# zrjer/Sparse-Matrix-Factorization-Library

Hardware: AMD Instinct MI355X
Metric: numeric-factorization GFLOP/s (supernodal Cholesky) (higher is better)
Workload: dtype f64; 1 GPU; 3D 7-point Laplacian 128^3 SPD Cholesky fp64, geometric ND, devSlotSize 8694792192; n=2097152, nnz_input=8339456, nsuper=35419, factor_doubles=3787034536, parallelism=single GPU, grid_rule=BASELINE config

## Files before the change

### sparse-matrix-factorization-library_amd/csrc/sf_chol_plan.hip

```cpp
#include <sparseframe_hip.h>

#include <algorithm>
#include <time.h>
#include <cmath>
#include <cstdio>
#include <cstdlib>
#include <cstring>
#include <string>
#include <vector>

#include "sf_plan_internal.h"
#include "sf_symbolic.h"

static bool elapsed_ms(float* ms, hipEvent_t a, hipEvent_t b) {
    if (hipEventElapsedTime(ms, a, b) == hipSuccess) return true;
    (void)hipGetLastError();
    return false;
}

extern "C" {

int sf_device_count(void) {
    int n = 0;
    if (hipGetDeviceCount(&n) != hipSuccess) return 0;
// ... 206 lines not shown
                break;
            case 1: sf::launch_trsm(p->d_trsm + L.first, L.count, p->d_Lsx, pc.pivinv, st); break;
            case 7: {
                const int g = (int)L.first;
                const int upto = p->ooc_wait.empty() ? g - 2 : p->ooc_wait[(size_t)g];
                for (int w = std::max(0, g - 2); w <= upto && w < g; ++w) {
                    std::unique_lock<std::mutex> lk(p->dl_mu);
                    p->dl_cv.wait(lk, [&] { return p->dl_abort || p->dl_group_left[(size_t)w].load() <= 0; });
                    if (p->dl_abort) return SF_ERR_HIP;
                }
                if (g >= 2 && p->ooc_buf > 0) {
                    const size_t off = (size_t)(g & 1) * (size_t)p->ooc_buf, nb = (size_t)p->ooc_buf * sizeof(double);
                    HIP_TRY(hipMemsetAsync(p->d_Lsx + off, 0, nb, st));
                    if (p->lu) HIP_TRY(hipMemsetAsync(p->d_Lsx + p->xC + off, 0, nb, st));
                }
                if (p->ooc_top_mode >= 1)
                    for (const auto& z : p->ooc_zero[(size_t)g]) {
                        HIP_TRY(hipMemsetAsync(p->d_Lsx + z.first, 0, (size_t)z.second * sizeof(double), st));
                        if (p->lu) HIP_TRY(hipMemsetAsync(p->d_Lsx + p->xC + z.first, 0, (size_t)z.second * sizeof(double), st));
                    }
                assemble(p->d_loadmask + (size_t)g * (size_t)p->nsuper, st);
                break;
            }
            case 6: {
                int64_t lo, hi;
                launch_window(L, L.count, &lo, &hi);
                sf::launch_update_small(p->d_probs, p->d_stasks + L.first + lo, (int)(hi - lo), p->d_Lsx, p->d_relmap, st);
                break;
            }
            case 5:
                sf::launch_step(p->d_steps + L.first, L.count, p->lu ? 1 : 0, p->d_Lsx, p->d_flags, p->epoch, p->d_info, p->d_tinv,
                                p->d_info + 1 + L.ticket, pc, st);
                break;
            case 2:
            case 3:
            case 4: {
                int64_t w0, w1;
                launch_window(L, L.units, &w0, &w1);
                const uint32_t u0 = (uint32_t)w0, u1 = (uint32_t)w1;
                sf::launch_gemm(p->d_probs, p->d_gtasks + L.first, p->d_ktprefix + L.prefix_first, L.count, u0, u1,
                                L.kind == 3 ? 1 : 0, p->d_Lsx, p->d_relmap, p->gemm_dynamic ? p->d_info + 1 + L.ticket : nullptr, st,
                                (L.whole_tiles && !L.split) ? 1 : 0, 0);
                break;
            }
        }
        if (p->profiling) { kinds.push_back(L.kind); mark(); }
        if (p->dl_active) HIP_TRY(dl_publish(p, li + 1));
    }
    if (last && !p->capturing) HIP_TRY(hipEventRecord(p->ev1, st));
    HIP_TRY(hipGetLastError());
    if (p->profiling) {
        HIP_TRY(hipStreamSynchronize(st));
        if (first) {
            p->last_load_ms = p->last_panel_ms = p->last_update_ms = 0;
            for (double& v : p->last_kind_ms) v = 0;
        }
        float ms = 0;
        if (first && !evs.empty() && elapsed_ms(&ms, p->ev0, evs[0])) p->last_load_ms = ms;
        FILE* dump = nullptr;
        if (const char* path = getenv("SF_PROFILE_DUMP")) dump = fopen(path, first ? "w" : "a");
        if (dump && first) fprintf(dump, "launch,kind,tasks,units,flops,ms\n");
        for (size_t k = 0; k + 1 < evs.size(); ++k) {
            if (!elapsed_ms(&ms, evs[k], evs[k + 1])) continue;
            if (kinds[k] == 3) p->last_update_ms += ms; else if (kinds[k] != 6) p->last_panel_ms += ms;
            p->last_kind_ms[kinds[k]] += ms;
            if (dump) {
// ... 761 lines not shown
    if (!p || !name) return -1;
    const std::string k(name);
    if (k == "levels") return p->nlevels;
    if (k == "last_solve_ms") return p->last_solve_ms;
    if (k == "last_solve_many_ms") return p->last_solve_many_ms;
    if (k == "bytes_solve_many") return (double)p->bytes_solve_many;
    if (k == "solve_many_width") return (double)sf::SVM_W;
    if (k == "bytes_selinv") return (double)p->bytes_selinv;
    if (k == "last_selinv_ms") return p->last_selinv_ms;
    if (k == "flops_selinv") return p->flops_selinv;
    if (k == "selinv_valid") return (p->d_sel && p->sel_gen == p->factor_gen) ? 1.0 : 0.0;
    if (k == "perturbed_pivots") return (double)p->last_perturbed;
    if (k == "pivot_tol") return p->piv_tol;
    if (k == "last_to_host_ms") return p->last_to_host_ms;
    if (k == "download_pieces") return (double)p->dl_pieces.size();
    if (k == "top_doubles") return (double)p->top_size;
    if (k == "stored_doubles") return (double)p->xC;
    if (k == "launches") return (double)p->launches.size();
    if (k == "gemm_tasks") return (double)p->n_gemm_tasks;
    if (k == "update_pairs") return (double)p->n_pairs;
    if (k == "flops_exec") return p->flops_exec;
    if (k == "flops_update") return p->flops_update;
    if (k == "flops_panel_gemm") return p->flops_panel_gemm;
    if (k == "scatter_elems") return p->scatter_elems;
    if (k == "bytes_device") return (double)p->bytes_device;
    if (k == "last_ms") return p->last_ms;
    if (k == "last_load_ms") return p->last_load_ms;
    if (k == "last_panel_ms") return p->last_panel_ms;
    if (k == "last_update_ms") return p->last_update_ms;
    if (k == "last_potrf_ms") return p->last_kind_ms[0];
    if (k == "last_trsm_ms") return p->last_kind_ms[1];
    if (k == "last_inner_gemm_ms") return p->last_kind_ms[2];
    if (k == "last_outer_gemm_ms") return p->last_kind_ms[4];
    if (k == "last_step_ms") return p->last_kind_ms[5];
    if (k == "last_small_update_ms") return p->last_kind_ms[6];
    if (k == "flops_update_small") return p->flops_update_small;
    if (k == "flops_outer_gemm") return p->flops_outer_gemm;
    if (k == "flops_tiles") return p->flops_tiles;
    if (k == "flops_tiles_update") return p->flops_tiles_update;
    return -1;
}

}

void sf_solve_step_fwd(sf_chol_plan* p, size_t k, const double* base, int* sync, int* tickets, hipStream_t st) {
    const auto& s = p->solve_steps[k];
    const int32_t* piv = (p->lu && p->piv_tol > 0.0) ? p->d_piv : nullptr;
    const int unit = p->lu ? 1 : 0;
    int* tk = tickets + sf_chol_plan::SOLVE_TICKETS * k;
    if (s.small) {
        sf::launch_solve_small_fwd(p->d_solve + s.fwd_first, s.ndiag, base, p->d_Lsi, p->d_x, unit, piv, st);
    } else {
        sf::launch_solve_fwd(p->d_solve + s.fwd_first, s.fwd_count, s.big, base, p->d_Lsi, p->d_x, unit, piv, sync, tk, p->d_solve_sync, st);
    }
}

void sf_solve_step_bwd(sf_chol_plan* p, size_t k, const double* base, int* sync, int* tickets, hipStream_t st) {
    const auto& s = p->solve_steps[k];
    int* tk = tickets + sf_chol_plan::SOLVE_TICKETS * k;
    if (s.small) {
        sf::launch_solve_small_bwd(p->d_solve + s.bwd_first, s.ndiag, base, p->d_Lsi, p->d_x, st);
    } else if (p->solve_bwd_fused) {
        sf::launch_solve_bwd(p->d_solve + s.bwd_first, s.count, s.big, base, p->d_Lsi, p->d_x, sync, tk + 1, p->d_solve_sync, st, p->d_solveT);
    } else {
        sf::launch_solve_bwd(p->d_solve + s.bwd_first, s.nrows_tasks, 0, base, p->d_Lsi, p->d_x, sync, tk + 1, p->d_solve_sync, st);
        sf::launch_solve_bwd(p->d_solve + s.bwd_first + s.nrows_tasks, s.count - s.nrows_tasks, s.big, base, p->d_Lsi, p->d_x, sync, tk + 2,
                             p->d_solve_sync, st, p->d_solveT);
// ... 128 lines not shown
```

### sparse-matrix-factorization-library_amd/csrc/sf_kernels.h

```cpp
#pragma once
#include <hip/hip_runtime.h>
#include <cstdint>

#include <cstdlib>
static inline const char* sf_exp_env(const char* name) {
#ifdef SF_EXPERIMENTS
    return getenv(name);
#else
    (void)name;
    return nullptr;
#endif
}

namespace sf {

constexpr int NB = 64;
constexpr int OUTER_NB = 512;
constexpr int TRSM_ROWS = 256;
constexpr int ST_ROWS = 64;
constexpr int GEMM_BM = 128;
constexpr int GEMM_BN = 128;
constexpr int GEMM_BK = 16;
constexpr int GEMM_WAVES = 8;
constexpr int GEMM_THREADS = 64 * GEMM_WAVES;
// ... 54 lines not shown
};

struct StepTask {
    int64_t panel;
    int64_t xpanel;
    int32_t ld, J, diag, b;
    int32_t row0, nrows;
    int32_t flag;
    int32_t mode;
    int32_t slot;
    int32_t next_b;
    int32_t first_col;
    int32_t pad;
};

void launch_build_loadmap(const int64_t* Lp, const int32_t* Li, int32_t n, const int32_t* Super, const int32_t* SuperMap,
                          const int64_t* Lsip, const int32_t* Lsi, const int64_t* Lsxp, int64_t base, int skip_diag, int64_t* map, hipStream_t st);
void launch_loadmap_drop(const int64_t* drop, int64_t count, int64_t* map, hipStream_t st);
void launch_load_mapped(const double* Lx, const int64_t* map, int64_t nnz, double* Lsx, hipStream_t st);
void launch_load_panels(const int64_t* Lp, const int32_t* Li, const double* Lx, int32_t n,
                        const int32_t* Super, const int32_t* SuperMap, const int64_t* Lsip, const int32_t* Lsi,
                        const int64_t* Lsxp, double* Lsx, int skip_diag, const int8_t* load_mask, hipStream_t st);
void launch_potrf(const PotrfTask* tasks, int ntasks, double* Lsx, int* info, hipStream_t st);
void launch_getrf(const PotrfTask* tasks, int ntasks, double* Lsx, int64_t u_shift, int* info, PivotCtl pc, hipStream_t st);
struct FillTile { int64_t xp; int32_t nsrow, r0, c0, cb, ce; };
void launch_factor_hash(const int32_t* Super, const int64_t* Lsip, const int64_t* Xp, const int64_t* RefXp, int32_t nsuper,
                        const double* PL, const double* PU, int lu, int64_t total, unsigned long long* H, hipStream_t st);
void launch_lu_fill_u11(const FillTile* tiles, int64_t ntiles, double* PL, const double* PU, hipStream_t st);
void launch_pack_lu(const int32_t* Super, const int64_t* Lsip, const int64_t* Xp, const int64_t* RefXp, int32_t nsuper,
                    const double* PL, const double* PU, double* out, int64_t e_begin, int64_t e_end, hipStream_t st);
void launch_trsm(const TrsmTask* tasks, int ntasks, double* Lsx, const int32_t* pivinv, hipStream_t st);
void launch_step(const StepTask* tasks, int ntasks, int lu, double* Lsx, int* flags, int epoch, int* info, double* tinv, int* ticket,
                 PivotCtl pc, hipStream_t st);
void launch_build_relmaps(const GemmProb* probs, int nprobs, const int32_t* Lsi, int32_t* RelMap, hipStream_t st);

void launch_gemm(const GemmProb* probs, const GemmTask* tasks, const uint32_t* kt_prefix, int ntasks, uint32_t u_lo, uint32_t u_hi,
                 int mode, double* Lsx, const int32_t* RelMap, int* ticket, hipStream_t st, int whole_tiles = 0, int grid_cap = 0);

void launch_update_small(const GemmProb* probs, const GemmTask* tasks, int ntasks, double* Lsx, const int32_t* RelMap, hipStream_t st);

struct SolveTask {
    int64_t panel;
    int64_t rows;
    int32_t ld, diag, b;
    int32_t row0, nrows;
    int32_t first_col;
    int32_t flag;
    int32_t expect;
    int64_t tdiag;
};
void launch_solve_small_fwd(const SolveTask* t, int nt, const double* Lsx, const int32_t* Lsi, double* x, int unit, const int32_t* pivpos,
                            hipStream_t st);
void launch_solve_small_bwd(const SolveTask* t, int nt, const double* Lsx, const int32_t* Lsi, double* x, hipStream_t st);
void launch_solve_fwd(const SolveTask* t, int nt, int big, const double* Lsx, const int32_t* Lsi, double* x, int unit, const int32_t* pivpos,
                      int* sync, int* ticket, int* info, hipStream_t st);
void launch_solve_bwd(const SolveTask* t, int nt, int big, const double* Lsx, const int32_t* Lsi, double* x, int* sync, int* ticket, int* info,
                      hipStream_t st, const double* Tbase = nullptr);
void launch_solve_transpose_diag(const SolveTask* tasks, const int64_t* list, int64_t ntasks, const double* Lsx, double* T, hipStream_t st);

constexpr int SVM_W = 16;
void launch_solve_many_small_fwd(const SolveTask* t, int nt, const double* Lsx, const int32_t* Lsi, double* x, int unit,
                                 const int32_t* pivpos, hipStream_t st);
void launch_solve_many_small_bwd(const SolveTask* t, int nt, const double* Lsx, const int32_t* Lsi, double* x, hipStream_t st);
void launch_solve_many_fwd(const SolveTask* t, int nt, int big, const double* Lsx, const int32_t* Lsi, double* x, int unit,
                           const int32_t* pivpos, int* sync, int* ticket, int* info, hipStream_t st);
void launch_solve_many_bwd(const SolveTask* t, int nt, int big, const double* Lsx, const int32_t* Lsi, double* x, int* sync, int* ticket,
// ... 23 lines not shown
```

### sparse-matrix-factorization-library_amd/csrc/sf_kernels.hip

```cpp
#include "sf_kernels.h"
#include <cstdlib>
#include "sf_wave.h"

namespace sf {

typedef double double4_t __attribute__((ext_vector_type(4)));
typedef double double2_t __attribute__((ext_vector_type(2), aligned(8)));

__device__ __forceinline__ int lower_bound_i32(const int32_t* __restrict__ a, int n, int32_t key) {
    int lo = 0, hi = n;
    while (lo < hi) {
        const int mid = (lo + hi) >> 1;
        if (a[mid] < key) lo = mid + 1; else hi = mid;
    }
    return lo;
}

__global__ void __launch_bounds__(256)
k_load_panels(const int64_t* __restrict__ Lp, const int32_t* __restrict__ Li, const double* __restrict__ Lx, int32_t n,
              const int32_t* __restrict__ Super, const int32_t* __restrict__ SuperMap,
              const int64_t* __restrict__ Lsip, const int32_t* __restrict__ Lsi,
              const int64_t* __restrict__ Lsxp, double* __restrict__ Lsx, int skip_diag,
              const int8_t* __restrict__ load_mask) {
    const int32_t j = blockIdx.x * blockDim.x + threadIdx.x;
// ... 1597 lines not shown
        g_exp_stamps[(size_t)gridDim.x * 256 + blockIdx.x * 4 + 3] = wall_clock64();
    }
#endif
}

#ifndef SF_LU_STEP_WGS
#define SF_LU_STEP_WGS 3
#endif
#ifndef SF_GEMM_MIN_UNITS_DEFAULT
#define SF_GEMM_MIN_UNITS_DEFAULT 16
#endif
#ifndef SF_POTRF_PW
#define SF_POTRF_PW 16
#endif
constexpr int ST_ULD = ST_ROWS + 1;
constexpr int ST_KC = 32;
constexpr int ST_XLD = ST_ROWS + 16;
constexpr int ST_SPIN_LIMIT = 1 << 22;

#ifdef SF_EXP_STEP_STAMPS
__device__ unsigned long long* g_step_stamps = nullptr;
void exp_set_step_stamps(unsigned long long* p) { (void)hipMemcpyToSymbol(HIP_SYMBOL(g_step_stamps), &p, sizeof(p)); }
#define ST_STAMP(slot) do { if (is_diag && tid == 0 && g_step_stamps) g_step_stamps[slot] = wall_clock64(); } while (0)
#else
#define ST_STAMP(slot) do { } while (0)
#endif

__device__ __forceinline__ double ld_agent(const double* p) {
    return __hip_atomic_load(p, __ATOMIC_RELAXED, __HIP_MEMORY_SCOPE_AGENT);
}
__device__ __forceinline__ int ld_agent(const int* p) {
    return __hip_atomic_load(p, __ATOMIC_RELAXED, __HIP_MEMORY_SCOPE_AGENT);
}

template <bool LU>
__global__ void __launch_bounds__(256, LU ? SF_LU_STEP_WGS : 3)
k_step(const StepTask* __restrict__ tasks, double* __restrict__ Lsx, int* __restrict__ flags, int epoch, int* __restrict__ info,
       double* __restrict__ tinv, int* __restrict__ ticket, PivotCtl pc) {
    constexpr int SMEM = 2 * ST_KC * ST_XLD;
    __shared__ __attribute__((aligned(16))) double smem[SMEM];
    static_assert(NB == ST_ROWS && NB == 64, "one wavefront per 64 x 64 tile");
    static_assert(NB * ST_ULD <= SMEM && NB * NB + 4 * 256 <= SMEM, "phases must fit the LDS array");
    double* __restrict__ U = smem;
    double (*Dt)[NB] = reinterpret_cast<double (*)[NB]>(smem);

    __shared__ int s_ticket;
    const int tid = threadIdx.x, lane = tid & 63, wave = tid >> 6;
#ifdef SF_EXP_STEP_STAMPS
    const unsigned long long st_entry = wall_clock64();
#endif
    if (tid == 0) s_ticket = __hip_atomic_fetch_add(ticket, 1, __ATOMIC_RELAXED, __HIP_MEMORY_SCOPE_AGENT);
    __syncthreads();
    const StepTask t = tasks[__builtin_amdgcn_readfirstlane(s_ticket)];
    const bool is_pre = LU && (t.mode & 2);
    const bool is_diag = t.row0 == t.diag && !is_pre;
#ifdef SF_EXP_STEP_STAMPS
    if (is_diag && tid == 0 && g_step_stamps) g_step_stamps[0] = st_entry;
#endif
    ST_STAMP(1);
    const int fr = lane & 15, fk = lane >> 4;
    const int64_t ld = t.ld;
    const int b = t.b, nrows = t.nrows;
    const int nhp = ((is_pre ? t.diag - NB : t.diag) - t.J) / NB;
    double* __restrict__ Ag = Lsx + t.panel + t.row0 + (int64_t)t.diag * ld;
    const double* __restrict__ Dg = Lsx + t.xpanel + t.diag + (int64_t)t.diag * ld;

    double4_t acc[4];
#pragma unroll
    for (int a = 0; a < 4; ++a) acc[a] = (double4_t){0.0, 0.0, 0.0, 0.0};

    if (nhp > 0) {
        double (*Xs)[ST_KC][ST_XLD] = reinterpret_cast<double (*)[ST_KC][ST_XLD]>(smem);
        const int nch = 2 * nhp;
        const int prow = 2 * (tid & 31), pk0 = tid >> 5;
        const double* __restrict__ xp = Lsx + t.xpanel + t.diag + (int64_t)t.J * ld + ((prow < b) ? prow : 0);
        const double* __restrict__ yp = Lsx + t.panel + t.row0 + (int64_t)(t.J + fk) * ld + min(16 * wave + fr, nrows - 1);
        const int nhalf = 2 * nch;
        double2_t rx[2][4];
        double fy[4][4];
        auto load_x = [&](int sel, int h) __attribute__((always_inline)) {
            const int hc = min(h, nch - 1);
#pragma unroll
            for (int q = 0; q < 4; ++q) rx[sel][q] = *reinterpret_cast<const double2_t*>(xp + (int64_t)(hc * ST_KC + pk0 + 8 * q) * ld);
        };
        auto store_x = [&](int buf, int sel) __attribute__((always_inline)) {
#pragma unroll
            for (int q = 0; q < 4; ++q) *reinterpret_cast<double2_t*>(&Xs[buf][pk0 + 8 * q][prow]) = rx[sel][q];
        };
        auto load_y = [&](int slot, int hh) __attribute__((always_inline)) {
            const int hc = min(hh, nhalf - 1);
#pragma unroll
            for (int kk = 0; kk < 4; ++kk) fy[slot][kk] = yp[(int64_t)(hc * (ST_KC / 2) + 4 * kk) * ld];
        };
        auto compute = [&](int par, int h) __attribute__((always_inline)) {
            load_y((2 * par + 3) & 3, 2 * h + 3);
#pragma unroll
            for (int kk = 0; kk < 8; ++kk) {
                double a[4];
#pragma unroll
                for (int q = 0; q < 4; ++q) a[q] = Xs[par][4 * kk + fk][16 * q + fr];
                if (kk == 0) store_x(par ^ 1, par ^ 1);
                if (kk == 1) load_x(par ^ 1, h + 3);
                if (kk == 4) load_y(2 * par, 2 * h + 4);
#pragma unroll
                for (int q = 0; q < 4; ++q) acc[q] = __builtin_amdgcn_mfma_f64_16x16x4f64(a[q], fy[2 * par + (kk >> 2)][kk & 3], acc[q], 0, 0, 0);
            }
        };
        load_x(0, 0);
        load_x(1, 1);
        load_y(0, 0);
        load_y(1, 1);
        load_y(2, 2);
        store_x(0, 0);
        load_x(0, 2);
        __syncthreads();
        for (int hp = 0; hp < nhp; ++hp) {
            compute(0, 2 * hp);
            __syncthreads();
            compute(1, 2 * hp + 1);
            __syncthreads();
        }
    }

    if (is_pre) {
        double* __restrict__ Dw = Lsx + t.xpanel + t.diag + (int64_t)t.diag * ld;
// ... 34 lines not shown
#pragma unroll
            for (int i = 0; i < 16; ++i) {
                const int k = 16 * wave + i;
                if (lane > k) U[k * ST_ULD + lane] = (lane < b && k < b) ? blk[i] : 0.0;
            }
#pragma unroll
            for (int i = 0; i < 16; ++i) blk[i] = Dg[lc + (int64_t)min(16 * wave + i, b - 1) * ld];
#pragma unroll
            for (int i = 0; i < 16; ++i) {
                const int k = 16 * wave + i;
                if (lane >= k) U[lane * ST_ULD + k] = (lane < b && k < b) ? blk[i] : ((lane == k) ? 1.0 : 0.0);
            }
        }
        if (nhp > 0) {
            __syncthreads();
            const int ci = 16 * wave + fr;
#pragma unroll
            for (int q = 0; q < 4; ++q)
#pragma unroll
                for (int r = 0; r < 4; ++r) {
                    const int cj = 16 * q + fk + 4 * r;
                    if (ci < b && cj < b) U[cj * ST_ULD + ci] -= acc[q][r];
                }
        }
    } else if (is_diag) {
        const int ci = 16 * wave + fr;
#pragma unroll
        for (int q = 0; q < 4; ++q)
#pragma unroll
            for (int r = 0; r < 4; ++r) {
                const int cj = 16 * q + fk + 4 * r;
                const int cic = min(ci, nrows - 1), cjc = min(cj, b - 1);
                double v = (ci == cj) ? 1.0 : 0.0;
                const double av = Ag[cic + (int64_t)cjc * ld];
                if (ci < nrows && cj < b && cj <= ci) v = av - acc[q][r];
                U[cj * ST_ULD + ci] = v;
            }
    }

    if (LU && is_diag) {
        __shared__ int s_piv[NB], s_pos[NB];
        if (tid < NB) { s_pos[tid] = -1; s_piv[tid] = tid; }
        __syncthreads();
        ST_STAMP(2);
        bool bad = false, active = lane < b;
        int np = 0, pos = lane;
        bool nat_all = true;
#pragma unroll 1
        for (int q = 0; q < NB / 16; ++q) {
            const int c0 = 16 * q;
            if (wave == 0) {
                double a[16];
#pragma unroll
                for (int u = 0; u < 16; ++u) a[u] = U[(c0 + u) * ST_ULD + lane];
                bool done = false;
                if (nat_all) {
                    done = getrf_panel_natural<16>(a, lane, c0, b, pc.tol, pc.eps);
                    if (done) {
                        if (lane >= c0 && lane < c0 + 16) { active = false; s_piv[lane] = lane; }
                    } else {
#pragma unroll
                        for (int u = 0; u < 16; ++u) a[u] = U[(c0 + u) * ST_ULD + lane];
                    }
                }
                if (!done) {
                    nat_all = false;
                    getrf_panel_wave<true, 16>(a, lane, c0, b, pc.tol, pc.eps, bad, np, pos, active, s_piv);
// ... 242 lines not shown
            double dv[NB * NB / 256], tv[4];
#pragma unroll
            for (int i = 0; i < NB * NB / 256; ++i) {
                const int e = tid + 256 * i, k = e / NB, j = e % NB;
                dv[i] = ld_agent(Dg + min(j, b - 1) + (int64_t)min(k, b - 1) * ld);
            }
#pragma unroll
            for (int i = 0; i < 4; ++i) tv[i] = ld_agent(tsrc + tid + 256 * i);
#pragma unroll
            for (int i = 0; i < NB * NB / 256; ++i) {
                const int e = tid + 256 * i, k = e / NB, j = e % NB;
                Dt[k][j] = (j < b && k < j) ? dv[i] : 0.0;
            }
#pragma unroll
            for (int i = 0; i < 4; ++i) Tl[tid + 256 * i] = tv[i];
        }
        __syncthreads();
        const int ci = 16 * wave + fr;
#pragma unroll
        for (int q = 0; q < 4; ++q) {
            if (16 * q >= b) break;
            double4_t x = (double4_t){0.0, 0.0, 0.0, 0.0};
#pragma unroll
            for (int sg = 0; sg < 4; ++sg)
                x = __builtin_amdgcn_mfma_f64_16x16x4f64(Tl[q * 256 + (4 * sg + fk) * 16 + fr], rt[q][sg], x, 0, 0, 0);
#pragma unroll
            for (int qq = q + 1; qq < 4; ++qq)
#pragma unroll
                for (int sg = 0; sg < 4; ++sg)
                    rt[qq] = __builtin_amdgcn_mfma_f64_16x16x4f64(-Dt[16 * q + 4 * sg + fk][16 * qq + fr], x[sg], rt[qq], 0, 0, 0);
#pragma unroll
            for (int r = 0; r < 4; ++r) {
                const int cj = 16 * q + fk + 4 * r;
                if (ci < nrows && cj < b) Ag[ci + (int64_t)cj * ld] = x[r];
            }
            if (!LU && t.next_b > 0) {
                __syncthreads();
#pragma unroll
                for (int r = 0; r < 4; ++r) Dt[16 * q + fk + 4 * r][ci] = x[r];
            }
        }
        if (!LU && t.next_b > 0) {
            __syncthreads();
            double* __restrict__ Dn = Lsx + t.panel + t.row0 + (int64_t)t.row0 * ld;
            const int nb = t.next_b;
            for (int ct = 0; ct <= wave; ++ct) {
                double4_t d = (double4_t){0.0, 0.0, 0.0, 0.0};
#pragma unroll 4
                for (int sg = 0; sg < 16; ++sg)
                    d = __builtin_amdgcn_mfma_f64_16x16x4f64(Dt[4 * sg + fk][16 * ct + fr], Dt[4 * sg + fk][ci], d, 0, 0, 0);
                double old[4];
#pragma unroll
                for (int r = 0; r < 4; ++r) {
                    const int cj = 16 * ct + fk + 4 * r;
                    old[r] = Dn[min(ci, nb - 1) + (int64_t)min(cj, nb - 1) * ld];
                }
#pragma unroll
                for (int r = 0; r < 4; ++r) {
                    const int cj = 16 * ct + fk + 4 * r;
                    if (ci < nb && cj <= ci) Dn[ci + (int64_t)cj * ld] = old[r] - d[r];
                }
            }
        }
    }
}

void launch_step(const StepTask* tasks, int ntasks, int lu, double* Lsx, int* flags, int epoch, int* info, double* tinv, int* ticket,
                 PivotCtl pc, hipStream_t st) {
    if (ntasks <= 0) return;
    if (lu) hipLaunchKernelGGL(k_step<true>, dim3(ntasks), dim3(256), 0, st, tasks, Lsx, flags, epoch, info, tinv, ticket, pc);
    else hipLaunchKernelGGL(k_step<false>, dim3(ntasks), dim3(256), 0, st, tasks, Lsx, flags, epoch, info, tinv, ticket, pc);
}

__global__ void __launch_bounds__(256)
k_update_small(const GemmProb* __restrict__ probs, const GemmTask* __restrict__ tasks, int ntasks,
               double* __restrict__ Lsx, const int32_t* __restrict__ RelMap) {
    const int lane = threadIdx.x & 63;
    const int ti = __builtin_amdgcn_readfirstlane(blockIdx.x * 4 + (threadIdx.x >> 6));
    if (ti >= ntasks) return;
    const GemmTask tk = tasks[ti];
    const GemmProb pb = probs[tk.prob];
    const int fr = lane & 15, fk = lane >> 4;
    const int ci0 = tk.tm * SU_TM, cj0 = tk.tn * SU_TN;
    const int M = pb.M, N = pb.N, K = pb.K;
    const int64_t lda = pb.lda;
    const double* __restrict__ yq[4];
    const double* __restrict__ xq[2];
#pragma unroll
    for (int q = 0; q < 4; ++q) yq[q] = Lsx + pb.y_off + min(ci0 + 16 * q + fr, M - 1);
#pragma unroll
    for (int q = 0; q < 2; ++q) xq[q] = Lsx + pb.x_off + min(cj0 + 16 * q + fr, N - 1);

    double4_t acc[2][4];
#pragma unroll
    for (int a = 0; a < 2; ++a)
#pragma unroll
        for (int c = 0; c < 4; ++c) acc[a][c] = (double4_t){0.0, 0.0, 0.0, 0.0};

    const int nkk = (K + 3) >> 2;
    for (int kk0 = 0; kk0 < nkk; kk0 += 8) {
        double fa[8][2], fb[8][4];
#pragma unroll
        for (int kk = 0; kk < 8; ++kk) {
            const int k = 4 * (kk0 + kk) + fk;
// ... 161 lines not shown
```

### sparse-matrix-factorization-library_amd/csrc/sf_plan_build.hip

```cpp
#include <sparseframe_hip.h>

#include <algorithm>
#include <time.h>
#include <cmath>
#include <cstdio>
#include <cstdlib>
#include <cstring>
#include <vector>

#include "sf_plan_internal.h"
#include "sf_symbolic.h"

static thread_local double* t_offer_ptr = nullptr;
static thread_local size_t t_offer_bytes = 0;
extern "C" void sf_plan_offer_factor_buffer(double* ptr, size_t bytes) { t_offer_ptr = ptr; t_offer_bytes = bytes; }

struct PlanInput {
    sf_long n = 0, nsuper = 0;
    const sf_long *Super = nullptr, *SuperMap = nullptr, *Lsip = nullptr, *Lsi = nullptr, *Lsxp = nullptr;
    const sf_long *Lp = nullptr, *Li = nullptr, *Up = nullptr, *Ui = nullptr;
    bool lu = false;
    int device = 0;
    bool dry = false;
    const int32_t* phase_in = nullptr;
    int load_top = 1, rank = 0, nranks = 1;
    const uint32_t* top_mask = nullptr;
    const double* root_cum = nullptr;
    const int32_t* ooc_group = nullptr;
    int ooc_ngroups = 0, ooc_top_mode = 0;

    sf_long nscol(sf_long s) const { return Super[s + 1] - Super[s]; }
    sf_long nsrow(sf_long s) const { return Lsip[s + 1] - Lsip[s]; }
    bool ooc() const { return ooc_group != nullptr && ooc_ngroups > 1; }
    int sides() const { return lu ? 2 : 1; }
};

static bool exp_on(const char* name) {
    const char* env = sf_exp_env(name);
    return !(env && atoi(env) == 0);
}

struct PlanKnobs {
    bool trace = false;
    int su_maxk = sf::SU_MAXK;
    int64_t fuse_max = 32 * sf::GEMM_GRID;
    bool lookahead = true;
    bool use_graph = false;
    bool top_owner = false;
    bool solve_diagT = true, solve_bwd_ahead = true, solve_bwd_fused = true, solve_fwd_ahead = true, solve_fwd_far_first = true;
    int solve_far_wgs = 512, solve_far_groups = 8;
    int dl_workers = DL_WORKERS_DEFAULT, dl_workers_fresh = DL_WORKERS_FRESH;
    bool dl_host_wait = true;
    int64_t dl_slot = DL_SLOT_DEFAULT;
    bool dl_2d = true;
    bool dl_lu_pack = false;
    bool stream_priority = true;
    bool gemm_dynamic = true;
    double piv_tol = 0.0, piv_perturb = 0.0;
};

static PlanKnobs read_knobs() {
    PlanKnobs k;
    k.trace = getenv("SF_TRACE") != nullptr;
    if (const char* env = sf_exp_env("SF_SU_MAXK")) k.su_maxk = atoi(env);
    if (const char* env = getenv("SF_FUSE_MAX")) k.fuse_max = strtoll(env, nullptr, 10);
    if (const char* env = getenv("SF_LOOKAHEAD")) k.lookahead = atoi(env) != 0;
    if (const char* env = getenv("SF_GRAPH")) k.use_graph = atoi(env) != 0;
    if (const char* env = getenv("SF_TOP_OWNER")) k.top_owner = atoi(env) != 0;
    k.solve_diagT = exp_on("SF_SOLVE_DIAGT");
    k.solve_bwd_ahead = exp_on("SF_SOLVE_BWD_AHEAD");
    k.solve_bwd_fused = exp_on("SF_SOLVE_BWD_FUSED");
    k.solve_fwd_ahead = exp_on("SF_SOLVE_FWD_AHEAD");
    k.solve_fwd_far_first = exp_on("SF_SOLVE_FWD_FAR_FIRST");
    if (const char* env = sf_exp_env("SF_SOLVE_FAR_WGS")) k.solve_far_wgs = std::max(1, atoi(env));
    if (const char* env = sf_exp_env("SF_SOLVE_FAR_GROUPS")) k.solve_far_groups = std::max(1, std::min(64, atoi(env)));
    if (const char* env = getenv("SF_DL_WORKERS")) k.dl_workers = k.dl_workers_fresh = std::max(1, std::min(DL_WORKERS_MAX, atoi(env)));
    k.dl_host_wait = exp_on("SF_DL_HOST_WAIT");
    if (const char* env = getenv("SF_DL_SLOT_MB")) k.dl_slot = (int64_t)std::max(1, atoi(env)) << 17;
    k.dl_2d = exp_on("SF_DL_2D");
    if (const char* env = sf_exp_env("SF_DL_LU_PACK")) k.dl_lu_pack = atoi(env) != 0;
    k.stream_priority = exp_on("SF_STREAM_PRIORITY");
    k.gemm_dynamic = exp_on("SF_GEMM_DYNAMIC");
    if (const char* env = getenv("SF_LU_PIVOT_TOL")) {
        k.piv_tol = std::min(1.0, std::max(0.0, atof(env)));
        if (k.piv_tol > 0.0) k.piv_perturb = 1.4901161193847656e-08;
    }
    if (const char* env = getenv("SF_LU_PERTURB")) k.piv_perturb = std::max(0.0, atof(env));
    return k;
}

struct Layout {
    std::vector<int64_t> XP;
    std::vector<uint32_t> gmask;
    int64_t ushift = 0;
    uint32_t all_ranks = 1;
    int rank = 0;
    int group_idx(uint32_t m) const { return __builtin_popcount(m & ((1u << rank) - 1u)); }
};
// ... 456 lines not shown
        const int dnext = diag + sf::NB;
        for (sf_long s : LS.sn) {
            const int nscol = (int)in.nscol(s), nsrow = (int)in.nsrow(s);
            if (dnext >= nscol) continue;
            const int bn = std::min(sf::NB, nscol - dnext);
            steps.push_back(StepTask{XP[s], XP[s] + ushift, nsrow, J, dnext, bn, dnext, bn, -1, 2, 0, 0, (int32_t)in.Super[s], 0});
            sw.pre_updated[(size_t)s] = jo * 16 + ti + 1;
        }
    }
    size_t si = 0;
    for (sf_long s : LS.sn) {
        const int nscol = (int)in.nscol(s), nsrow = (int)in.nsrow(s);
        const int32_t fl = flag_of[si], sl = slot_of[si];
        ++si;
        if (fl < 0) continue;
        const int b = std::min(sf::NB, nscol - diag);
        for (int r = diag + b; r < nsrow; r += sf::ST_ROWS) {
            const int nr = std::min(sf::ST_ROWS, nsrow - r);
            if (!lu) {
                const int nb = (r < std::min(nscol, J + sf::OUTER_NB)) ? std::min(sf::NB, nscol - r) : 0;
                steps.push_back(StepTask{XP[s], XP[s], nsrow, J, diag, b, r, nr, fl, 0, sl, nb, (int32_t)in.Super[s], 0});
            } else {
                steps.push_back(StepTask{XP[s], XP[s] + ushift, nsrow, J, diag, b, r, nr, fl, 0, sl, 0, (int32_t)in.Super[s], 0});
                steps.push_back(StepTask{XP[s] + ushift, XP[s], nsrow, J, diag, b, r, nr, fl, 1, sl, 0, (int32_t)in.Super[s], 0});
            }
        }
    }
    if ((int64_t)steps.size() > d0) {
        p.launches.push_back(Launch{5, d0, (int)(steps.size() - d0)});
        p.launches.back().ticket = p.n_tickets++;
    }
    T.max_diag_tasks = std::max<int64_t>(T.max_diag_tasks, (int64_t)slot_of.size());
    return SF_OK;
}

static void three_launch_step(const PlanInput& in, const Layout& lay, const LevelSet& LS, PlanTables& T, sf_chol_plan& p, int J, int diag) {
    const std::vector<int64_t>& XP = lay.XP;
    const int64_t ushift = lay.ushift;
    const int64_t p0 = (int64_t)T.potrf.size(), t0 = (int64_t)T.trsm.size(), g0 = (int64_t)T.gtasks.size();
    for (sf_long s : LS.sn) {
        const int nscol = (int)in.nscol(s), nsrow = (int)in.nsrow(s);
        if (diag >= nscol) continue;
        const int b = std::min(sf::NB, nscol - diag);
        if (diag > J) {
            GemmProb g{};
            g.lda = nsrow; g.ldc = nsrow;
            g.M = nsrow - diag; g.N = b; g.K = diag - J;
            const int64_t src = XP[s] + diag + (int64_t)J * nsrow;
            const int64_t dst = XP[s] + diag + (int64_t)diag * nsrow;
            const int32_t first = push_sides(in, lay, T, g, src, dst);
            for (int32_t id = first; id < (int32_t)T.probs.size(); ++id) {
                p.flops_panel_gemm += (double)g.N * (g.N + 1) * g.K + 2.0 * (g.M - g.N) * (double)g.N * g.K;
                add_tiles(T, p, id);
            }
        }
        T.potrf.push_back(PotrfTask{XP[s], nsrow, diag, b, (int32_t)in.Super[s]});
        const int below = diag + b;
        for (int r = below; r < nsrow; r += sf::TRSM_ROWS) {
            const int nr = std::min(sf::TRSM_ROWS, nsrow - r);
            if (!in.lu) {
                T.trsm.push_back(TrsmTask{XP[s], XP[s], nsrow, diag, b, r, nr, 0, (int32_t)in.Super[s], 0});
            } else {
                T.trsm.push_back(TrsmTask{XP[s], XP[s] + ushift, nsrow, diag, b, r, nr, 0, (int32_t)in.Super[s], 0});
                T.trsm.push_back(TrsmTask{XP[s] + ushift, XP[s], nsrow, diag, b, r, nr, 1, (int32_t)in.Super[s], 0});
            }
        }
// ... 74 lines not shown
        stamp_share(p.launches.back(), LS, shared);
        p.launches.back().flops = level_small_flops;
    }
}

static int schedule_set(const PlanInput& in, const PlanKnobs& kn, const Layout& lay, const LevelSet& LS, SweepState& sw, PlanTables& T,
                        sf_chol_plan& p) {
    if (LS.ph == 1 && !sw.split_set) { p.launch_split = p.launches.size(); sw.split_set = true; }
    while (in.ooc() && LS.group > sw.ooc_open) p.launches.push_back(Launch{7, (int64_t)++sw.ooc_open, 0});
    const bool shared = set_is_shared(in, LS);
    sf_long maxcol = 0;
    for (sf_long s : LS.sn) maxcol = std::max(maxcol, in.nscol(s));
    const int nouter = (int)((maxcol + sf::OUTER_NB - 1) / sf::OUTER_NB);
    const bool ahead = shared && p.lookahead && LS.share_cnt > 1;
    constexpr int KT_BLOCK = sf::OUTER_NB / sf::GEMM_BK;
    for (int jo = 0; jo < nouter; ++jo) {
        const int J = jo * sf::OUTER_NB;
        if (jo > 0 && !ahead) outer_gemm(in, lay, LS, T, p, J, 0, -1, shared);
        if (shared) {
            reduce_point(in, lay, LS, p, jo, ahead);
            if (ahead && jo > 0) outer_gemm(in, lay, LS, T, p, J, (jo - 1) * KT_BLOCK, jo * KT_BLOCK, false);
        }
        const int ninner = sf::OUTER_NB / sf::NB;
        bool block_fused = false;
        for (int ti = 0; ti < ninner; ++ti) {
            const int diag = J + ti * sf::NB;
            if (diag >= maxcol) break;
            int64_t step_wgs = 0;
            for (sf_long s : LS.sn) {
                const int64_t nscol = in.nscol(s), nsrow = in.nsrow(s);
                if (diag < nscol) step_wgs += 1 + in.sides() * ((nsrow - std::min<int64_t>(nscol, diag + sf::NB) + sf::ST_ROWS - 1) / sf::ST_ROWS);
            }
            if (ti == 0) block_fused = step_wgs <= kn.fuse_max;
            if (!block_fused) three_launch_step(in, lay, LS, T, p, J, diag);
            else if (int rc = fused_step(in, lay, LS, sw, T, p, jo, ti, diag)) return rc;
        }
        const bool owner_block = shared && !p.segments.empty() && p.segments.back().owner_gi >= 0;
        if (owner_block) p.segments.back().lc = p.launches.size();
        for (sf_long s : LS.sn)
            if (J < in.nscol(s)) T.blk_ready[T.blk_first[s] + jo] = p.launches.size() + (owner_block ? 1 : 0);
        if (ahead && jo + 2 < nouter) outer_gemm(in, lay, LS, T, p, J + 2 * sf::OUTER_NB, 0, (jo + 1) * KT_BLOCK, true);
    }
    schur_updates(in, kn, lay, LS, T, p);
    return SF_OK;
}

static int schedule_factorization(const PlanInput& in, const PlanKnobs& kn, const Layout& lay, const std::vector<LevelSet>& sets,
                                  PlanTables& T, sf_chol_plan& p) {
    T.blk_first.assign(in.nsuper + 1, 0);
    for (sf_long s = 0; s < in.nsuper; ++s) T.blk_first[s + 1] = T.blk_first[s] + (in.nscol(s) + sf::OUTER_NB - 1) / sf::OUTER_NB;
    T.blk_ready.assign(T.blk_first[in.nsuper], 0);
    p.lookahead = kn.lookahead;
    p.use_graph = kn.use_graph;
    p.top_owner = kn.top_owner && !in.lu;
    SweepState sw;
    sw.pre_updated.assign(in.lu ? (size_t)std::max<sf_long>(in.nsuper, 1) : 0, -1);
    p.launch_split = 0;
    for (const LevelSet& LS : sets)
        if (int rc = schedule_set(in, kn, lay, LS, sw, T, p)) return rc;
    if (!sw.split_set) p.launch_split = p.launches.size();
    if (!p.segments.empty()) p.segments.back().l1 = p.launches.size();
    p.n_gemm_tasks = (int64_t)T.gtasks.size() + (int64_t)T.stasks.size();
    return SF_OK;
}

static void schedule_solve(const PlanInput& in, const PlanKnobs& kn, const Layout& lay, PlanTables& T, sf_chol_plan& p) {
// ... 747 lines not shown
```

### sparse-matrix-factorization-library_amd/csrc/sf_plan_internal.h

```cpp
#pragma once
#include <sparseframe_hip.h>

#include <algorithm>
#include <atomic>
#include <condition_variable>
#include <cstdio>
#include <cstdlib>
#include <memory>
#include <mutex>
#include <thread>
#include <utility>
#include <vector>

#include "sf_kernels.h"

using sf::GemmProb;
using sf::GemmTask;
using sf::PotrfTask;
using sf::TrsmTask;
using sf::StepTask;

struct Launch {
    int kind;
    int64_t first;
// ... 193 lines not shown
    int64_t* d_Lsip = nullptr;
    int32_t* d_Lsi = nullptr;
    int64_t* d_Lsxp = nullptr;
    double* d_Lsx = nullptr;
    int* d_info = nullptr;
    int n_tickets = 0;
    bool gemm_dynamic = true;

    PotrfTask* d_potrf = nullptr;
    TrsmTask* d_trsm = nullptr;
    StepTask* d_steps = nullptr;
    int* d_flags = nullptr;
    double* d_tinv = nullptr;
    int epoch = 0;
    std::vector<uint64_t> h_hash;
    int hash_epoch = -1;
    GemmProb* d_probs = nullptr;
    GemmTask* d_gtasks = nullptr;
    GemmTask* d_stasks = nullptr;
    uint32_t* d_ktprefix = nullptr;
    int32_t* d_relmap = nullptr;

    std::vector<Launch> launches;
    int nlevels = 0;
    int64_t n_gemm_tasks = 0, n_pairs = 0;
    double flops_tiles = 0, flops_tiles_update = 0;
    double flops_update_small = 0;
    double flops_exec = 0, flops_update = 0, scatter_elems = 0, flops_panel_gemm = 0, flops_outer_gemm = 0;
    size_t bytes_device = 0;
    bool values_set = false;

    bool profiling = false;
    double last_ms = 0, last_load_ms = 0, last_panel_ms = 0, last_update_ms = 0;
    double last_kind_ms[8] = {0, 0, 0, 0, 0, 0, 0, 0};
    int last_status = SF_OK;

    std::vector<int64_t> h_Lsip, h_Lsxp;
    std::vector<int32_t> h_Super;
    std::vector<int> level_of;
};


int sf_dl_begin(sf_chol_plan* p, double* host_out);
extern "C" int sf_plan_panel_hashes(sf_chol_plan* p, const uint64_t** out);
int sf_dl_end(sf_chol_plan* p);
int sf_plan_import_from(sf_chol_plan* dst, sf_chol_plan* const* parts, int nparts);
int sf_seg_begin(sf_chol_plan* p, sf_long k, void** dptr, sf_long* count);
void* sf_plan_stream2(sf_chol_plan* p);
int sf_seg_reduced(sf_chol_plan* p, sf_long k);
int sf_seg_finish(sf_chol_plan* p, sf_long k);
int sf_seg_is_owner_segment(const sf_chol_plan* p, sf_long k);
int sf_seg_bcast_begin(sf_chol_plan* p, sf_long k, void** dptr, sf_long* count);
int sf_seg_bcast_finish(sf_chol_plan* p, sf_long k);
int sf_seg_early(const sf_chol_plan* p, sf_long k);
```

Baseline: 52690 GFLOP/s.

## Chain all inner panel steps of an outer block into one flag-synchronized launch

Adds a chained variant of the fused panel step kernel. It processes all inner 64-column steps of a 512-column outer block in a single launch. Workgroups wait on per-row-block agent-scope flags, bumped after each step, instead of relying on kernel boundaries between steps. The planner uses it for mid-sized Cholesky blocks, selected by a work-group count window. The aim is to remove per-step launch overhead and serialization. The cost is spin-waiting, atomic-scope loads and stores on panel data, and a deadlock risk if dependent workgroups are not resident.

```diff
diff --git a/sparse-matrix-factorization-library_amd/csrc/sf_chol_plan.hip b/sparse-matrix-factorization-library_amd/csrc/sf_chol_plan.hip
--- a/sparse-matrix-factorization-library_amd/csrc/sf_chol_plan.hip
+++ b/sparse-matrix-factorization-library_amd/csrc/sf_chol_plan.hip
@@ -262,6 +262,10 @@
                 sf::launch_step(p->d_steps + L.first, L.count, p->lu ? 1 : 0, p->d_Lsx, p->d_flags, p->epoch, p->d_info, p->d_tinv,
                                 p->d_info + 1 + L.ticket, pc, st);
                 break;
+            case 8:
+                sf::launch_step_chain(p->d_steps + L.first, L.count, p->d_Lsx, p->d_flags, p->epoch, p->d_info, p->d_tinv,
+                                      p->d_info + 1 + L.ticket, st);
+                break;
             case 2:
             case 3:
             case 4: {
@@ -1089,7 +1093,7 @@
     if (k == "last_trsm_ms") return p->last_kind_ms[1];
     if (k == "last_inner_gemm_ms") return p->last_kind_ms[2];
     if (k == "last_outer_gemm_ms") return p->last_kind_ms[4];
-    if (k == "last_step_ms") return p->last_kind_ms[5];
+    if (k == "last_step_ms") return p->last_kind_ms[5] + p->last_kind_ms[8];
     if (k == "last_small_update_ms") return p->last_kind_ms[6];
     if (k == "flops_update_small") return p->flops_update_small;
     if (k == "flops_outer_gemm") return p->flops_outer_gemm;
diff --git a/sparse-matrix-factorization-library_amd/csrc/sf_kernels.h b/sparse-matrix-factorization-library_amd/csrc/sf_kernels.h
--- a/sparse-matrix-factorization-library_amd/csrc/sf_kernels.h
+++ b/sparse-matrix-factorization-library_amd/csrc/sf_kernels.h
@@ -110,6 +110,8 @@
 void launch_trsm(const TrsmTask* tasks, int ntasks, double* Lsx, const int32_t* pivinv, hipStream_t st);
 void launch_step(const StepTask* tasks, int ntasks, int lu, double* Lsx, int* flags, int epoch, int* info, double* tinv, int* ticket,
                  PivotCtl pc, hipStream_t st);
+void launch_step_chain(const StepTask* tasks, int ntasks, double* Lsx, int* flags, int epoch, int* info, double* tinv, int* ticket,
+                       hipStream_t st);
 void launch_build_relmaps(const GemmProb* probs, int nprobs, const int32_t* Lsi, int32_t* RelMap, hipStream_t st);
 
 void launch_gemm(const GemmProb* probs, const GemmTask* tasks, const uint32_t* kt_prefix, int ntasks, uint32_t u_lo, uint32_t u_hi,
diff --git a/sparse-matrix-factorization-library_amd/csrc/sf_kernels.hip b/sparse-matrix-factorization-library_amd/csrc/sf_kernels.hip
--- a/sparse-matrix-factorization-library_amd/csrc/sf_kernels.hip
+++ b/sparse-matrix-factorization-library_amd/csrc/sf_kernels.hip
@@ -1653,8 +1653,13 @@
 __device__ __forceinline__ int ld_agent(const int* p) {
     return __hip_atomic_load(p, __ATOMIC_RELAXED, __HIP_MEMORY_SCOPE_AGENT);
 }
-
-template <bool LU>
+__device__ __forceinline__ void st_agent(double* p, double v) {
+    __hip_atomic_store(p, v, __ATOMIC_RELAXED, __HIP_MEMORY_SCOPE_AGENT);
+}
+template <bool CHAIN> __device__ __forceinline__ double ld_step(const double* p) { return CHAIN ? ld_agent(p) : *p; }
+template <bool CHAIN> __device__ __forceinline__ void st_step(double* p, double v) { if (CHAIN) st_agent(p, v); else *p = v; }
+
+template <bool LU, bool CHAIN = false>
 __global__ void __launch_bounds__(256, LU ? SF_LU_STEP_WGS : 3)
 k_step(const StepTask* __restrict__ tasks, double* __restrict__ Lsx, int* __restrict__ flags, int epoch, int* __restrict__ info,
        double* __restrict__ tinv, int* __restrict__ ticket, PivotCtl pc) {
@@ -1682,7 +1687,27 @@
     const int fr = lane & 15, fk = lane >> 4;
     const int64_t ld = t.ld;
     const int b = t.b, nrows = t.nrows;
-    const int nhp = ((is_pre ? t.diag - NB : t.diag) - t.J) / NB;
+    static_assert(!(LU && CHAIN), "chain launches are Cholesky only");
+    const int nhp = (CHAIN && is_diag) ? 0 : ((is_pre ? t.diag - NB : t.diag) - t.J) / NB;
+    const int cstep = CHAIN ? (t.diag - t.J) / NB : 0;
+    const int wtag = (int)((unsigned)epoch * 16u);
+    int* __restrict__ words = flags + (CHAIN ? t.pad : 0);
+    const int wlo = CHAIN ? (t.row0 - t.J) / NB : 0;
+    if (CHAIN && cstep > 0) {
+        if (tid == 0) {
+            const int whi = (t.row0 + t.nrows - 1 - t.J) / NB;
+            int spins = 0;
+            for (int k = 0; k < 3; ++k) {
+                const int w = k == 0 ? wlo : k == 1 ? whi : cstep;
+                while (ld_agent(words + w) != wtag + cstep) {
+                    __builtin_amdgcn_s_sleep(16);
+                    if (++spins > ST_SPIN_LIMIT) { atomicOr(info, 2); break; }
+                }
+            }
+            asm volatile("s_waitcnt vmcnt(0)" ::: "memory");
+        }
+        __syncthreads();
+    }
     double* __restrict__ Ag = Lsx + t.panel + t.row0 + (int64_t)t.diag * ld;
     const double* __restrict__ Dg = Lsx + t.xpanel + t.diag + (int64_t)t.diag * ld;
 
@@ -1702,7 +1727,11 @@
         auto load_x = [&](int sel, int h) __attribute__((always_inline)) {
             const int hc = min(h, nch - 1);
 #pragma unroll
-            for (int q = 0; q < 4; ++q) rx[sel][q] = *reinterpret_cast<const double2_t*>(xp + (int64_t)(hc * ST_KC + pk0 + 8 * q) * ld);
+            for (int q = 0; q < 4; ++q) {
+                const double* __restrict__ xq = xp + (int64_t)(hc * ST_KC + pk0 + 8 * q) * ld;
+                if (CHAIN) rx[sel][q] = (double2_t){ld_agent(xq), ld_agent(xq + 1)};
+                else rx[sel][q] = *reinterpret_cast<const double2_t*>(xq);
+            }
         };
         auto store_x = [&](int buf, int sel) __attribute__((always_inline)) {
 #pragma unroll
@@ -1711,7 +1740,7 @@
         auto load_y = [&](int slot, int hh) __attribute__((always_inline)) {
             const int hc = min(hh, nhalf - 1);
 #pragma unroll
-            for (int kk = 0; kk < 4; ++kk) fy[slot][kk] = yp[(int64_t)(hc * (ST_KC / 2) + 4 * kk) * ld];
+            for (int kk = 0; kk < 4; ++kk) fy[slot][kk] = ld_step<CHAIN>(yp + (int64_t)(hc * (ST_KC / 2) + 4 * kk) * ld);
         };
         auto compute = [&](int par, int h) __attribute__((always_inline)) {
             load_y((2 * par + 3) & 3, 2 * h + 3);
@@ -1812,7 +1841,7 @@
                 const int cj = 16 * q + fk + 4 * r;
                 const int cic = min(ci, nrows - 1), cjc = min(cj, b - 1);
                 double v = (ci == cj) ? 1.0 : 0.0;
-                const double av = Ag[cic + (int64_t)cjc * ld];
+                const double av = ld_step<CHAIN>(Ag + cic + (int64_t)cjc * ld);
                 if (ci < nrows && cj < b && cj <= ci) v = av - acc[q][r];
                 U[cj * ST_ULD + ci] = v;
             }
@@ -2121,7 +2150,7 @@
 #pragma unroll
             for (int r = 0; r < 4; ++r) {
                 const int cj = 16 * q + fk + 4 * r;
-                if (ci < nrows && cj < b) Ag[ci + (int64_t)cj * ld] = x[r];
+                if (ci < nrows && cj < b) st_step<CHAIN>(Ag + ci + (int64_t)cj * ld, x[r]);
             }
             if (!LU && t.next_b > 0) {
                 __syncthreads();
@@ -2142,15 +2171,20 @@
 #pragma unroll
                 for (int r = 0; r < 4; ++r) {
                     const int cj = 16 * ct + fk + 4 * r;
-                    old[r] = Dn[min(ci, nb - 1) + (int64_t)min(cj, nb - 1) * ld];
+                    old[r] = ld_step<CHAIN>(Dn + min(ci, nb - 1) + (int64_t)min(cj, nb - 1) * ld);
                 }
 #pragma unroll
                 for (int r = 0; r < 4; ++r) {
                     const int cj = 16 * ct + fk + 4 * r;
-                    if (ci < nb && cj <= ci) Dn[ci + (int64_t)cj * ld] = old[r] - d[r];
+                    if (ci < nb && cj <= ci) st_step<CHAIN>(Dn + ci + (int64_t)cj * ld, old[r] - d[r]);
                 }
             }
         }
+    }
+    if (CHAIN && b == NB) {
+        asm volatile("s_waitcnt vmcnt(0)" ::: "memory");
+        __syncthreads();
+        if (tid == 0) __hip_atomic_store(words + wlo, wtag + cstep + 1, __ATOMIC_RELAXED, __HIP_MEMORY_SCOPE_AGENT);
     }
 }
 
@@ -2159,6 +2193,13 @@
     if (ntasks <= 0) return;
     if (lu) hipLaunchKernelGGL(k_step<true>, dim3(ntasks), dim3(256), 0, st, tasks, Lsx, flags, epoch, info, tinv, ticket, pc);
     else hipLaunchKernelGGL(k_step<false>, dim3(ntasks), dim3(256), 0, st, tasks, Lsx, flags, epoch, info, tinv, ticket, pc);
+}
+
+void launch_step_chain(const StepTask* tasks, int ntasks, double* Lsx, int* flags, int epoch, int* info, double* tinv, int* ticket,
+                       hipStream_t st) {
+    if (ntasks <= 0) return;
+    hipLaunchKernelGGL((k_step<false, true>), dim3(ntasks), dim3(256), 0, st, tasks, Lsx, flags, epoch, info, tinv, ticket,
+                       PivotCtl{0.0, 0.0, nullptr, nullptr, nullptr});
 }
 
 __global__ void __launch_bounds__(256)
diff --git a/sparse-matrix-factorization-library_amd/csrc/sf_plan_build.hip b/sparse-matrix-factorization-library_amd/csrc/sf_plan_build.hip
--- a/sparse-matrix-factorization-library_amd/csrc/sf_plan_build.hip
+++ b/sparse-matrix-factorization-library_amd/csrc/sf_plan_build.hip
@@ -44,6 +44,8 @@
     bool trace = false;
     int su_maxk = sf::SU_MAXK;
     int64_t fuse_max = 32 * sf::GEMM_GRID;
+    bool chain = true;
+    int64_t chain_min = 600, chain_max = 2000;
     bool lookahead = true;
     bool use_graph = false;
     bool top_owner = false;
@@ -64,6 +66,9 @@
     k.trace = getenv("SF_TRACE") != nullptr;
     if (const char* env = sf_exp_env("SF_SU_MAXK")) k.su_maxk = atoi(env);
     if (const char* env = getenv("SF_FUSE_MAX")) k.fuse_max = strtoll(env, nullptr, 10);
+    if (const char* env = getenv("SF_CHAIN")) k.chain = atoi(env) != 0;
+    if (const char* env = getenv("SF_CHAIN_MIN")) k.chain_min = strtoll(env, nullptr, 10);
+    if (const char* env = getenv("SF_CHAIN_MAX")) k.chain_max = strtoll(env, nullptr, 10);
     if (const char* env = getenv("SF_LOOKAHEAD")) k.lookahead = atoi(env) != 0;
     if (const char* env = getenv("SF_GRAPH")) k.use_graph = atoi(env) != 0;
     if (const char* env = getenv("SF_TOP_OWNER")) k.top_owner = atoi(env) != 0;
@@ -586,6 +591,55 @@
     }
     T.max_diag_tasks = std::max<int64_t>(T.max_diag_tasks, (int64_t)slot_of.size());
     return SF_OK;
+}
+
+static void chain_block(const PlanInput& in, const Layout& lay, const LevelSet& LS, PlanTables& T, sf_chol_plan& p, int jo, sf_long maxcol) {
+    const int J = jo * sf::OUTER_NB, ninner = sf::OUTER_NB / sf::NB;
+    const std::vector<int64_t>& XP = lay.XP;
+    std::vector<StepTask>& steps = T.steps;
+    const int64_t d0 = (int64_t)steps.size();
+    std::vector<int32_t> wbase(LS.sn.size(), -1), flag_of(LS.sn.size()), slot_of(LS.sn.size());
+    for (size_t si = 0; si < LS.sn.size(); ++si) {
+        const sf_long s = LS.sn[si];
+        if (J >= in.nscol(s)) continue;
+        wbase[si] = T.n_flags;
+        T.n_flags += (int32_t)((in.nsrow(s) - J + sf::NB - 1) / sf::NB);
+    }
+    int32_t nslot = 0;
+    for (int ti = 0; ti < ninner; ++ti) {
+        const int diag = J + ti * sf::NB;
+        if (diag >= maxcol) break;
+        for (size_t si = 0; si < LS.sn.size(); ++si) {
+            const sf_long s = LS.sn[si];
+            const int nscol = (int)in.nscol(s), nsrow = (int)in.nsrow(s);
+            flag_of[si] = slot_of[si] = -1;
+            if (diag >= nscol) continue;
+            const int b = std::min(sf::NB, nscol - diag);
+            flag_of[si] = T.n_flags++;
+            slot_of[si] = nslot++;
+            steps.push_back(StepTask{XP[s], XP[s], nsrow, J, diag, b, diag, b, flag_of[si], 0, slot_of[si], 0, (int32_t)in.Super[s], wbase[si]});
+            if (ti > 0) p.flops_panel_gemm += (double)b * (b + 1) * (diag - J) + 2.0 * (nsrow - diag - b) * (double)b * (diag - J);
+        }
+        for (int pass = 0; pass < 2; ++pass)
+            for (size_t si = 0; si < LS.sn.size(); ++si) {
+                if (flag_of[si] < 0) continue;
+                const sf_long s = LS.sn[si];
+                const int nscol = (int)in.nscol(s), nsrow = (int)in.nsrow(s);
+                const int b = std::min(sf::NB, nscol - diag);
+                for (int r = diag + b; r < nsrow; r += sf::ST_ROWS) {
+                    const int nr = std::min(sf::ST_ROWS, nsrow - r);
+                    const int nb = (r < std::min(nscol, J + sf::OUTER_NB)) ? std::min(sf::NB, nscol - r) : 0;
+                    const bool critical = nb > 0 && r == diag + sf::NB;
+                    if (critical != (pass == 0)) continue;
+                    steps.push_back(StepTask{XP[s], XP[s], nsrow, J, diag, b, r, nr, flag_of[si], 0, slot_of[si], nb, (int32_t)in.Super[s], wbase[si]});
+                }
+            }
+    }
+    if ((int64_t)steps.size() > d0) {
+        p.launches.push_back(Launch{8, d0, (int)(steps.size() - d0)});
+        p.launches.back().ticket = p.n_tickets++;
+    }
+    T.max_diag_tasks = std::max<int64_t>(T.max_diag_tasks, nslot);
 }
 
 static void three_launch_step(const PlanInput& in, const Layout& lay, const LevelSet& LS, PlanTables& T, sf_chol_plan& p, int J, int diag) {
@@ -726,6 +780,10 @@
                 if (diag < nscol) step_wgs += 1 + in.sides() * ((nsrow - std::min<int64_t>(nscol, diag + sf::NB) + sf::ST_ROWS - 1) / sf::ST_ROWS);
             }
             if (ti == 0) block_fused = step_wgs <= kn.fuse_max;
+            if (ti == 0 && block_fused && kn.chain && !in.lu && in.nranks == 1 && step_wgs >= kn.chain_min && step_wgs <= kn.chain_max) {
+                chain_block(in, lay, LS, T, p, jo, maxcol);
+                break;
+            }
             if (!block_fused) three_launch_step(in, lay, LS, T, p, J, diag);
             else if (int rc = fused_step(in, lay, LS, sw, T, p, jo, ti, diag)) return rc;
         }
diff --git a/sparse-matrix-factorization-library_amd/csrc/sf_plan_internal.h b/sparse-matrix-factorization-library_amd/csrc/sf_plan_internal.h
--- a/sparse-matrix-factorization-library_amd/csrc/sf_plan_internal.h
+++ b/sparse-matrix-factorization-library_amd/csrc/sf_plan_internal.h
@@ -249,7 +249,7 @@
 
     bool profiling = false;
     double last_ms = 0, last_load_ms = 0, last_panel_ms = 0, last_update_ms = 0;
-    double last_kind_ms[8] = {0, 0, 0, 0, 0, 0, 0, 0};
+    double last_kind_ms[9] = {0, 0, 0, 0, 0, 0, 0, 0, 0};
     int last_status = SF_OK;
 
     std::vector<int64_t> h_Lsip, h_Lsxp;
```

Result: no change. 52780 GFLOP/s, median of 6 (+0.2%).
